# davidmilligan/MLVFS

Hardware: AMD Instinct MI355X
Metric: Mpix/s, 3584x1320 14-bit unpack+badpix+cs5x5+stripes (fused, stream resident in HBM) (higher is better)
Workload: dtype u16/int32

## Files before the change

mlvfs_amd/csrc/k_frame_dev.h:

```cpp
#pragma once
#include "clip.h"
#include <cstdlib>
#include <map>
#include <mutex>
#include <vector>
#include <algorithm>
#include <cstdio>
#include <type_traits>

typedef short mlv_pk16 __attribute__((ext_vector_type(2)));
__device__ __forceinline__ int mlv_min_(int a, int b) { return min(a, b); }
__device__ __forceinline__ int mlv_max_(int a, int b) { return max(a, b); }
__device__ __forceinline__ mlv_pk16 mlv_min_(mlv_pk16 a, mlv_pk16 b) { return __builtin_elementwise_min(a, b); }
__device__ __forceinline__ mlv_pk16 mlv_max_(mlv_pk16 a, mlv_pk16 b) { return __builtin_elementwise_max(a, b); }
#define MLV_NET_FN __device__ __forceinline__
#define mlv_mn(a, b) mlv_min_((a), (b))
#define mlv_mx(a, b) mlv_max_((a), (b))
#include "median_nets.h"


namespace mlv {

constexpr int TCW = FRAME_TCW;
constexpr int TCH = FRAME_TCH;
// ... 770 lines not shown
    for (int c = 0; c < STRIP + 2; c++) {
        const int a = plane[row_top][col_left + c], b = plane[row_top + 1][col_left + c], d = plane[row_top + 2][col_left + c];
        lo[c] = min(min(a, b), d);
        hi[c] = max(max(a, b), d);
        mi[c] = med3i(a, b, d);
    }
#pragma unroll
    for (int c = 0; c < STRIP; c++)
        med[c] = med3i(max(max(lo[c], lo[c + 1]), lo[c + 2]), med3i(mi[c], mi[c + 1], mi[c + 2]),
                       min(min(hi[c], hi[c + 1]), hi[c + 2]));
}

__device__ __forceinline__ void strip_median5(const int (*plane)[PW], int row_top, int col_left, int (&med)[STRIP])
{
#pragma unroll
    for (int c = 0; c < STRIP; c++) {
        const int v[5] = { plane[row_top][col_left + c + 1], plane[row_top + 1][col_left + c],
                           plane[row_top + 1][col_left + c + 1], plane[row_top + 1][col_left + c + 2],
                           plane[row_top + 2][col_left + c + 1] };
        int o[1];
        mlv_median5(v, o);
        med[c] = o[0];
    }
}

template <bool FAST>
__device__ __forceinline__ uint32_t stripe_px(uint32_t p, int coef, int black16, int white16)
{
    if (FAST) {
        const int a = (int)p - black16;
        const int v = (int)p + (__mul24(a, coef - 65536) >> 16);
        return (a > 64) ? (uint32_t)min(v, white16) : p;
    }
    if (coef == 0 || (int)p <= black16 + 64) return p;
    const long long num = (long long)((int)p - black16) * coef + ((long long)black16 << 16);
    if (((long long)white16 << 16) < num) return (uint32_t)white16;
    return (uint32_t)(int)(num / 65536) & 0xFFFFu;
}

template <bool FAST>
__device__ __forceinline__ void stripe_strip(uint32_t (&top)[STRIP], uint32_t (&bot)[STRIP], const int (&coef)[8], int black16, int white16)
{
#pragma unroll
    for (int c = 0; c < STRIP; c++) {
        const int p0 = (2 * c) & 7, p1 = (2 * c + 1) & 7;
        top[c] = stripe_px<FAST>(top[c] & 0xFFFFu, coef[p0], black16, white16) |
                 (stripe_px<FAST>(top[c] >> 16, coef[p1], black16, white16) << 16);
        bot[c] = stripe_px<FAST>(bot[c] & 0xFFFFu, coef[p0], black16, white16) |
                 (stripe_px<FAST>(bot[c] >> 16, coef[p1], black16, white16) << 16);
    }
}

template <bool MASK = true>
__device__ __forceinline__ uint32_t stripe_pair(uint32_t x, int d0, int d1, uint32_t black_pk, uint32_t white_pk)
{
    typedef unsigned short upk16 __attribute__((ext_vector_type(2)));
    const mlv_pk16 a = __builtin_bit_cast(mlv_pk16, x) - __builtin_bit_cast(mlv_pk16, black_pk);
    const mlv_pk16 c64 = { 64, 64 }, s15 = { 15, 15 };
    const int p0 = __mul24((int)a.x, d0), p1 = __mul24((int)a.y, d1);
    const uint32_t delta = __builtin_amdgcn_perm((uint32_t)p1, (uint32_t)p0, 0x07060302u);
    uint32_t dm = delta;
    if (MASK) dm &= __builtin_bit_cast(uint32_t, (c64 - a) >> s15);
    const upk16 v = __builtin_bit_cast(upk16, x) + __builtin_bit_cast(upk16, dm);
    return __builtin_bit_cast(uint32_t, __builtin_elementwise_min(v, __builtin_bit_cast(upk16, white_pk)));
}

template <bool MASK = true>
__device__ __forceinline__ void stripe_strip_pk(uint32_t (&top)[STRIP], uint32_t (&bot)[STRIP], const int (&coef)[8], int black16, int white16)
{
    const uint32_t black_pk = (uint32_t)black16 * 0x10001u, white_pk = (uint32_t)white16 * 0x10001u;
#pragma unroll
    for (int c = 0; c < STRIP; c++) {
        const int d0 = coef[(2 * c) & 7] - 65536, d1 = coef[(2 * c + 1) & 7] - 65536;
        if ((d0 | d1) == 0) {
            typedef unsigned short upk16 __attribute__((ext_vector_type(2)));
            top[c] = __builtin_bit_cast(uint32_t, __builtin_elementwise_min(__builtin_bit_cast(upk16, top[c]), __builtin_bit_cast(upk16, white_pk)));
            bot[c] = __builtin_bit_cast(uint32_t, __builtin_elementwise_min(__builtin_bit_cast(upk16, bot[c]), __builtin_bit_cast(upk16, white_pk)));
            continue;
        }
        top[c] = stripe_pair<MASK>(top[c], d0, d1, black_pk, white_pk);
        bot[c] = stripe_pair<MASK>(bot[c], d0, d1, black_pk, white_pk);
    }
}



typedef const __attribute__((address_space(4))) FrameArgs *KArgs;
__device__ __forceinline__ KArgs cold_args()
{
    KArgs p = (KArgs)__builtin_amdgcn_kernarg_segment_ptr();
    asm volatile("" : "+s"(p));
    return p;
}


template <int BPP>
__device__ __forceinline__ void item_tile_offsets(const ItemLane &L, int l_row, int w, uint32_t &pre_a, uint32_t &pre_b)
{
    constexpr uint32_t GB = (uint32_t)BPP;
    const uint32_t pitch = (uint32_t)(w >> 3) * GB;
    const uint32_t rowoff = __umul24((uint32_t)(2 * l_row), pitch) + 16u;
    pre_a = rowoff + ((uint32_t)((L.xoff_a >> 3) * (int)GB) & L.amask);
    pre_b = rowoff + ((uint32_t)((L.xoff_b >> 3) * (int)GB) & L.amask) + L.boff;
}
template <int BPP, int VEC, class LANE>
__device__ __forceinline__ void issue_tile_rows_pre(uint32_t (&r0)[4], uint32_t (&r1)[4], const uint8_t *frame, unsigned bytes, uint32_t pre_a, uint32_t pre_b,
                                                    LANE lane_of, int w, int h, int tx0, int ty0, int new0)
{
    constexpr uint32_t GB = (uint32_t)BPP;
    const uint32_t pitch = (uint32_t)(w >> 3) * GB;
    const int ybase = ty0 - 2 * HC + 2 * new0;
    uint32_t oa0, ob0, oa1, ob1, S = 0;
    if (VEC != 2 && tx0 >= 8 && tx0 + 2 * TCW + 8 <= w && ybase + 2 * TCH <= h) {
        S = (uint32_t)ybase * pitch + (uint32_t)(tx0 >> 3) * GB - 16u;
        oa0 = pre_a;
        ob0 = pre_b;
        oa1 = oa0 + pitch;
        ob1 = ob0 + pitch;
    } else {
        int l_row;
        const ItemLane L = lane_of(l_row);
        const int y = ybase + 2 * l_row;
        const int gmax = (w >> 3) - 1, g0 = tx0 >> 3;
        const uint32_t ga = __umul24((uint32_t)min(g0 + (L.xoff_a >> 3), gmax), GB);
        const uint32_t gb = __umul24((uint32_t)max(min(g0 + (L.xoff_b >> 3), gmax), 0), GB);
        const uint32_t row0 = __umul24((uint32_t)min(y, h - 1), pitch), row1 = __umul24((uint32_t)min(y + 1, h - 1), pitch);
        oa0 = (row0 + ga) & L.amask; ob0 = ((row0 + gb) & L.amask) + L.boff;
        oa1 = (row1 + ga) & L.amask; ob1 = ((row1 + gb) & L.amask) + L.boff;
        asm volatile("" : "+v"(oa0), "+v"(ob0));
    }
    const mlv_i32x4 rs = frame_rsrc(frame + S, bytes - S);
    const mlv_u32x2 a0 = mlv_rbl_x2(rs, (int)oa0, 0, AUX_DEFAULT), b0 = mlv_rbl_x2(rs, (int)ob0, 0, AUX_DEFAULT);
    const mlv_u32x2 a1 = mlv_rbl_x2(rs, (int)oa1, 0, AUX_DEFAULT), b1 = mlv_rbl_x2(rs, (int)ob1, 0, AUX_DEFAULT);
    r0[0] = a0.x; r0[1] = a0.y; r0[2] = b0.x; r0[3] = b0.y;
    r1[0] = a1.x; r1[1] = a1.y; r1[2] = b1.x; r1[3] = b1.y;
}
template <int BPP, int VEC>
__device__ __forceinline__ void issue_tile_rows(uint32_t (&r0)[4], uint32_t (&r1)[4], const uint8_t *frame, unsigned bytes, const ItemLane &L, int l_row,
                                                int w, int h, int tx0, int ty0, int new0)
{
    uint32_t pre_a, pre_b;
    item_tile_offsets<BPP>(L, l_row, w, pre_a, pre_b);
    issue_tile_rows_pre<BPP, VEC>(r0, r1, frame, bytes, pre_a, pre_b, [&](int &row) { row = l_row; return L; }, w, h, tx0, ty0, new0);
}

struct OutArgs {
    const uint2 *e2d;
    uint8_t *dst;
    size_t dst_stride;
    int stripes, coef_pk, coef_fast, white;
    int co[8];
};
__device__ __forceinline__ OutArgs out_args(KArgs kt)
{
    OutArgs o;
    o.e2d = kt->e2d; o.dst = kt->dst; o.dst_stride = kt->dst_stride;
    o.stripes = kt->stripes; o.coef_pk = kt->coef_pk; o.coef_fast = kt->coef_fast; o.white = kt->white;
#pragma unroll
    for (int i = 0; i < 8; i++) o.co[i] = kt->coef[i];
    return o;
}

__device__ __forceinline__ void put_rb(uint32_t &top, uint32_t &bot, uint32_t ur, uint32_t ub, unsigned long long m)
{
    asm("s_mov_b64 vcc, %4\n\t"
        "v_cndmask_b32_sdwa %0, %0, %2, vcc dst_sel:WORD_0 dst_unused:UNUSED_PRESERVE src0_sel:WORD_0 src1_sel:WORD_0\n\t"
        "v_cndmask_b32_sdwa %1, %1, %3, vcc dst_sel:WORD_1 dst_unused:UNUSED_PRESERVE src0_sel:WORD_1 src1_sel:WORD_0"
        : "+v"(top), "+v"(bot) : "v"(ur), "v"(ub), "s"(m) : "vcc");
}
__device__ __forceinline__ unsigned long long lanes_gt(int a, int b) { return __builtin_amdgcn_sicmp(a, b, 38); }
__device__ __forceinline__ unsigned long long lanes_ge(int a, int b) { return __builtin_amdgcn_sicmp(a, b, 39); }
__device__ __forceinline__ unsigned long long lanes_lt(int a, int b) { return __builtin_amdgcn_sicmp(a, b, 40); }

struct NoSmem {};
__device__ __forceinline__ bool smoothed_low(const int (&er)[STRIP], const int (&eb)[STRIP])
{
    const int lo = min(min(min(min(er[0], er[1]), er[2]), min(er[3], eb[0])), min(min(eb[1], eb[2]), eb[3]));
    return __any(lo < 7 * MLV_EV_RES);
}
template <int METHOD, bool PACKED, bool VECST, bool CLAMP, bool XM, bool ANYSTRIPES, bool BRIGHT, class SM, bool RAWREG = false>
__device__ __forceinline__ void strip_output_t(const SM &sm, const OutArgs &oa, int w, int h, int black, int f, int tx0, int ty0, int jj, int kk,
                                               unsigned long long msmooth, const int (&gev)[STRIP], int gev_off, const int (&er)[STRIP], const int (&eb)[STRIP], bool store,
                                               uint32_t *rtop = nullptr, uint32_t *rbot = nullptr)
{
    const int y = ty0 + 2 * jj, x = tx0 + 2 * STRIP * kk;
    uint32_t top[STRIP], bot[STRIP];
    auto read_raw = [&]() {
        if constexpr (RAWREG) {
#pragma unroll
            for (int c = 0; c < STRIP; c++) { top[c] = rtop[c]; bot[c] = rbot[c]; }
        } else {
            const uint4 v0 = *(const uint4 *)&sm.raw[2 * jj][2 * STRIP * kk];
            const uint4 v1 = *(const uint4 *)&sm.raw[2 * jj + 1][2 * STRIP * kk];
            top[0] = v0.x; top[1] = v0.y; top[2] = v0.z; top[3] = v0.w;
            bot[0] = v1.x; bot[1] = v1.y; bot[2] = v1.z; bot[3] = v1.w;
        }
    };
    if (METHOD == 0) read_raw();
    if (METHOD != 0) {
        const mlv_i32x4 rs_e2d = table_rsrc(oa.e2d, 8, E2D_RECORDS_EXT);
        int ur[STRIP], ub[STRIP], cr[STRIP], cb[STRIP];
        mlv_tab_u32x2 dr2[STRIP], db2[STRIP];
#pragma unroll
        for (int c = 0; c < STRIP; c++) {
            cr[c] = CLAMP ? min(max(er[c], 0), MLV_EV_MAX) : er[c];
            cb[c] = CLAMP ? min(max(eb[c], 0), MLV_EV_MAX) : eb[c];
            dr2[c] = mlv_sbl_x2(rs_e2d, cr[c] >> 5, 0, 0, AUX_DEFAULT);
            db2[c] = mlv_sbl_x2(rs_e2d, cb[c] >> 5, 0, 0, AUX_DEFAULT);
        }
        read_raw();
        asm volatile("" :: "v"(dr2[0]), "v"(dr2[1]), "v"(dr2[2]), "v"(dr2[3]), "v"(db2[0]), "v"(db2[1]), "v"(db2[2]), "v"(db2[3]));
#pragma unroll
        for (int c = 0; c < STRIP; c++) {
            ur[c] = (int)(__builtin_popcount(bfe_low_bits(dr2[c].y, (uint32_t)cr[c])) + dr2[c].x);
            ub[c] = (int)(__builtin_popcount(bfe_low_bits(db2[c].y, (uint32_t)cb[c])) + db2[c].x);
        }
#pragma unroll
        for (int c = 0; c < STRIP; c++) {
            unsigned long long okm = msmooth;
            if (!BRIGHT) okm &= lanes_ge((int)((uint32_t)gev[c] - (uint32_t)gev_off), 2 * MLV_EV_RES) & lanes_gt(er[c], MLV_EV_RES) & lanes_gt(eb[c], MLV_EV_RES);
            if (XM) okm &= lanes_ge(x + 2 * c, 4) & lanes_lt(x + 2 * c, w - 4);
            put_rb(top[c], bot[c], (uint32_t)ur[c], (uint32_t)ub[c], okm);
        }
    }
    if (oa.stripes) {
        const int black16 = (int)(uint16_t)black, white16 = (int)(uint16_t)oa.white;
        if (!ANYSTRIPES) stripe_strip_pk<CLAMP>(top, bot, oa.co, black16, white16);
        else if (PACKED && oa.coef_pk) stripe_strip_pk<true>(top, bot, oa.co, black16, white16);
        else if (oa.coef_fast) stripe_strip<true>(top, bot, oa.co, black16, white16);
        else stripe_strip<false>(top, bot, oa.co, black16, white16);
    }
    if constexpr (RAWREG) {
#pragma unroll
        for (int c = 0; c < STRIP; c++) { rtop[c] = top[c]; rbot[c] = bot[c]; }
    }
    if (store && y < h) {
        if (VECST) {
            if (x < w) {
                const uint32_t T = ((uint32_t)ty0 * (uint32_t)w + (uint32_t)tx0) * 2u;
                const mlv_i32x4 rs_out = frame_rsrc(oa.dst + (size_t)f * oa.dst_stride + T, (uint32_t)w * (uint32_t)h * 2u - T);
                const uint32_t vo = (__umul24((uint32_t)(2 * jj), (uint32_t)w) + 2 * STRIP * (uint32_t)kk) * 2u;
                const mlv_u32x4 vt = { top[0], top[1], top[2], top[3] }, vb = { bot[0], bot[1], bot[2], bot[3] };
                mlv_rbs_x4(vt, rs_out, (int)vo, 0, 2);
                if (y + 1 < h) mlv_rbs_x4(vb, rs_out, (int)vo, w * 2, 2);
            }
        } else {
            uint16_t *out = (uint16_t *)(oa.dst + (size_t)f * oa.dst_stride);
#pragma unroll 1
            for (int c = 0; c < STRIP; c++) {
                const int xc = x + 2 * c;
                if (xc < w) out[(size_t)y * w + xc] = (uint16_t)top[c];
                if (xc + 1 < w) out[(size_t)y * w + xc + 1] = (uint16_t)(top[c] >> 16);
                if (y + 1 < h) {
                    if (xc < w) out[(size_t)(y + 1) * w + xc] = (uint16_t)bot[c];
                    if (xc + 1 < w) out[(size_t)(y + 1) * w + xc + 1] = (uint16_t)(bot[c] >> 16);
                }
            }
        }
    }
}

template <int METHOD, bool PACKED, bool VECST, class SM>
__device__ __forceinline__ void strip_output(const SM &sm, const OutArgs &oa, int w, int h, int black, int f, int tx0, int ty0, int jj, int kk,
                                             unsigned long long msmooth, const int (&gev)[STRIP], int gev_off, const int (&er)[STRIP], const int (&eb)[STRIP], bool low_any, bool bright,
                                             bool store)
{
    const bool xm = tx0 < 4 || tx0 + 2 * TCW > w - 4;
    if (METHOD != 0 && !low_any && oa.stripes && smoothed_low(er, eb)) { low_any = true; bright = false; }
    if (oa.stripes && !(PACKED && oa.coef_pk)) {
        strip_output_t<METHOD, PACKED, VECST, true, true, true, false, SM>(sm, oa, w, h, black, f, tx0, ty0, jj, kk, msmooth, gev, gev_off, er, eb, store);
    } else if (low_any) {
        if (xm) strip_output_t<METHOD, PACKED, VECST, true, true, false, false, SM>(sm, oa, w, h, black, f, tx0, ty0, jj, kk, msmooth, gev, gev_off, er, eb, store);
        else strip_output_t<METHOD, PACKED, VECST, true, false, false, false, SM>(sm, oa, w, h, black, f, tx0, ty0, jj, kk, msmooth, gev, gev_off, er, eb, store);
    } else if (xm) {
        strip_output_t<METHOD, PACKED, VECST, false, true, false, false, SM>(sm, oa, w, h, black, f, tx0, ty0, jj, kk, msmooth, gev, gev_off, er, eb, store);
    } else {
        if (bright) strip_output_t<METHOD, PACKED, VECST, false, false, false, true, SM>(sm, oa, w, h, black, f, tx0, ty0, jj, kk, msmooth, gev, gev_off, er, eb, store);
        else strip_output_t<METHOD, PACKED, VECST, false, false, false, false, SM>(sm, oa, w, h, black, f, tx0, ty0, jj, kk, msmooth, gev, gev_off, er, eb, store);
    }
}

template <int N> using IntC = std::integral_constant<int, N>;
template <class F>
void with_layout(int method, bool packed, int vec, bool spread, F &&f)
{
    auto with_v = [&](auto M, auto P) {
        auto go = [&](auto V) { if (spread && M.value != 0) f(M, P, V, std::true_type{}); else f(M, P, V, std::false_type{}); };
        switch (vec) {
            case 1: return go(IntC<1>{});
            case 2: return go(IntC<2>{});
            case 3: if constexpr (P.value) return go(IntC<3>{}); break;
            case 4: if constexpr (P.value) return go(IntC<4>{}); break;
        }
        go(IntC<0>{});
    };
    auto with_p = [&](auto M) { if (packed) with_v(M, std::true_type{}); else with_v(M, std::false_type{}); };
    switch (method) {
        case 0: return with_p(IntC<0>{});
        case 2: return with_p(IntC<2>{});
        case 3: return with_p(IntC<3>{});
        case 5: return with_p(IntC<5>{});
    }
}

}
```

mlvfs_amd/csrc/k_frame_p.hip:

```cpp
#include "frame_plan.h"
#include "k_stream_dev.h"

namespace mlv {

constexpr int P_WAIT_MIN = 1, P_WAIT_MAX = 15;
template <bool SPREAD_>
struct __align__(16) SmemP {
    static constexpr bool SPREAD = SPREAD_;
    uint16_t raw[2 * RH][2 * TCW];
    uint32_t pk[PH][PW];
    int ge[RH][TCW];
    uint16_t t16[MLV_T16_N + (SPREAD_ ? 64 : 0)];
    uint32_t has_patch[PMAP_WORDS];
    uint32_t xchg[3][XCHG_WORDS];
    int unc[2];
    int low[2];
    int dim[2];
    int next_tile, next_end;
    int walk[5];
    int2 carry_at[256];
    uint4 carry_spare;
};

struct PGroup {
    mlv_pk16 s[4][5];
    mlv_pk16 p0[10], p1[10];
    mlv_pk16 q[6];
};
struct PNext { mlv_pk16 s0[5], s2[5], p0[10], q[6]; };

__device__ __forceinline__ mlv_pk16 as_pk(uint32_t v) { return __builtin_bit_cast(mlv_pk16, v); }
__device__ __forceinline__ uint32_t as_u(mlv_pk16 v) { return __builtin_bit_cast(uint32_t, v); }

__device__ __forceinline__ void pchain_group(const uint32_t (*pk)[PW], int row_top, int col_left, PGroup &g)
{
    mlv_pk16 col[4][5];
#pragma unroll
    for (int r = 0; r < 5; r++) {
        const uint4 v = *(const uint4 *)&pk[row_top + r][col_left];
        col[0][r] = as_pk(v.x); col[1][r] = as_pk(v.y); col[2][r] = as_pk(v.z); col[3][r] = as_pk(v.w);
    }
#pragma unroll
    for (int c = 0; c < 4; c++) mlv_sort5(col[c], g.s[c]);
    mlv_merge55(g.s[0], g.s[1], g.p0);
    mlv_merge55(g.s[2], g.s[3], g.p1);
}
__device__ __forceinline__ void pchain_fetch_lists(const PGroup &g, PNext &n)
{
#pragma unroll
    for (int i = 0; i < 5; i++) { n.s0[i] = dpp_next(g.s[0][i]); n.s2[i] = dpp_next(g.s[2][i]); }
#pragma unroll
    for (int i = 0; i < 10; i++) n.p0[i] = dpp_next(g.p0[i]);
}
__device__ __forceinline__ void pchain_fetch_window(const PGroup &g, PNext &n)
{
#pragma unroll
    for (int i = 0; i < 6; i++) n.q[i] = dpp_next(g.q[i]);
}
__device__ __forceinline__ void pchain_publish(const PGroup &g, uint32_t *x)
{
    uint4 *o = (uint4 *)x;
    o[0] = make_uint4(as_u(g.s[0][0]), as_u(g.s[0][1]), as_u(g.s[0][2]), as_u(g.s[0][3]));
    o[1] = make_uint4(as_u(g.s[0][4]), as_u(g.s[2][0]), as_u(g.s[2][1]), as_u(g.s[2][2]));
    o[2] = make_uint4(as_u(g.s[2][3]), as_u(g.s[2][4]), as_u(g.p0[0]), as_u(g.p0[1]));
    o[3] = make_uint4(as_u(g.p0[2]), as_u(g.p0[3]), as_u(g.p0[4]), as_u(g.p0[5]));
    o[4] = make_uint4(as_u(g.p0[6]), as_u(g.p0[7]), as_u(g.p0[8]), as_u(g.p0[9]));
    o[5] = make_uint4(as_u(g.q[0]), as_u(g.q[1]), as_u(g.q[2]), as_u(g.q[3]));
    *(uint2 *)&o[6] = make_uint2(as_u(g.q[4]), as_u(g.q[5]));
}
__device__ __forceinline__ void pchain_collect_lists(const uint32_t *x, PNext &n)
{
    const uint4 *o = (const uint4 *)x;
    const uint4 a0 = o[0], a1 = o[1], a2 = o[2], a3 = o[3], a4 = o[4];
    n.s0[0] = as_pk(a0.x); n.s0[1] = as_pk(a0.y); n.s0[2] = as_pk(a0.z); n.s0[3] = as_pk(a0.w); n.s0[4] = as_pk(a1.x);
    n.s2[0] = as_pk(a1.y); n.s2[1] = as_pk(a1.z); n.s2[2] = as_pk(a1.w); n.s2[3] = as_pk(a2.x); n.s2[4] = as_pk(a2.y);
    n.p0[0] = as_pk(a2.z); n.p0[1] = as_pk(a2.w); n.p0[2] = as_pk(a3.x); n.p0[3] = as_pk(a3.y); n.p0[4] = as_pk(a3.z);
    n.p0[5] = as_pk(a3.w); n.p0[6] = as_pk(a4.x); n.p0[7] = as_pk(a4.y); n.p0[8] = as_pk(a4.z); n.p0[9] = as_pk(a4.w);
}
__device__ __forceinline__ void pchain_collect_window(const uint32_t *x, PNext &n)
{
    const uint4 a5 = *(const uint4 *)(x + 20);
    const uint2 a6 = *(const uint2 *)(x + 24);
    n.q[0] = as_pk(a5.x); n.q[1] = as_pk(a5.y); n.q[2] = as_pk(a5.z); n.q[3] = as_pk(a5.w); n.q[4] = as_pk(a6.x); n.q[5] = as_pk(a6.y);
}
__device__ __forceinline__ void pchain_finish(const PGroup &g, const PNext &n, mlv_pk16 (&o)[STRIP])
{
    mlv_pk16 q1[6], t[1];
    mlv_quad_mid6(g.p1, n.p0, q1);
    mlv_final6of11(g.q, n.s0, t);  o[0] = t[0];
    mlv_final6of11(q1, g.s[1], t); o[1] = t[0];
    mlv_final6of11(q1, n.s2, t);   o[2] = t[0];
    mlv_final6of11(n.q, g.s[3], t); o[3] = t[0];
}
__device__ __forceinline__ bool pk_uncertain(const mlv_pk16 (&o)[STRIP])
{
    typedef unsigned short upk16 __attribute__((ext_vector_type(2)));
    const upk16 off = { 32769, 32769 }, two = { 2, 2 };
    upk16 m = __builtin_bit_cast(upk16, o[0]) + off;
#pragma unroll
    for (int c = 1; c < STRIP; c++) m = __builtin_elementwise_min(m, (upk16)(__builtin_bit_cast(upk16, o[c]) + off));
    return __builtin_bit_cast(uint32_t, __builtin_elementwise_min(m, two)) != 0x00020002u;
}

__device__ __forceinline__ uint32_t add3_u32(uint32_t a, uint32_t b, uint32_t c)
{
    uint32_t r;
    asm("v_add3_u32 %0, %1, %2, %3" : "=v"(r) : "v"(a), "v"(b), "v"(c));
    return r;
}
template <int NC, bool SPREAD>
__device__ __forceinline__ void cell_multi_pk_fast(const uint32_t *p0, const uint32_t *p1, int black, const uint16_t *t, int ref_r, int ref_b,
                                                   int (&ge)[NC], uint32_t (&pk)[NC])
{
    uint32_t fb[4 * NC], tv[4 * NC];
    const float fmagic = 8388608.0f + (float)black;
#pragma unroll
    for (int c = 0; c < NC; c++) {
        const uint32_t px[4] = { p0[2 * c], p0[2 * c + 1], p1[2 * c], p1[2 * c + 1] };
#pragma unroll
        for (int i = 0; i < 4; i++) fb[4 * c + i] = __float_as_uint(__uint_as_float(px[i] | 0x4B000000u) - fmagic);
    }
#pragma unroll
    for (int i = 0; i < 4 * NC; i++) tv[i] = *(const uint16_t *)((const char *)t + t16_offset<SPREAD>(fb[i]));
    uint32_t exr[NC], exb[NC], exg[NC];
#pragma unroll
    for (int c = 0; c < NC; c++) { exr[c] = fb[4 * c] >> 8; exb[c] = fb[4 * c + 3] >> 8; exg[c] = (fb[4 * c + 1] + fb[4 * c + 2]) >> 8; }
#pragma unroll
    for (int c = 0; c < NC; c += 2) {
        asm volatile("" :: "v"(exr[c]), "v"(exb[c]), "v"(exg[c]), "v"(exr[c + 1]), "v"(exb[c + 1]), "v"(exg[c + 1]));
    }
#pragma unroll
    for (int i = 0; i < 4 * NC; i += 8) {
        asm volatile("" :: "v"(tv[i]), "v"(tv[i + 1]), "v"(tv[i + 2]), "v"(tv[i + 3]), "v"(tv[i + 4]), "v"(tv[i + 5]), "v"(tv[i + 6]), "v"(tv[i + 7]));
    }
    uint32_t nref_r = 0u - (uint32_t)ref_r, nref_b = 0u - (uint32_t)ref_b;
    asm("" : "+v"(nref_r), "+v"(nref_b));
#pragma unroll
    for (int c = 0; c < NC; c++) {
        const uint32_t gb = add3_u32(exg[c], tv[4 * c + 1], tv[4 * c + 2]) >> 1;
        ge[c] = (int)(gb - (127u << 15));
        uint32_t ngr = nref_r - gb, ngb = nref_b - gb;
        pk[c] = as_u(__builtin_amdgcn_cvt_pk_i16((int)add3_u32(exr[c], tv[4 * c + 0], ngr), (int)add3_u32(exb[c], tv[4 * c + 3], ngb)));
    }
}

template <int NC>
__device__ __forceinline__ void cell_multi_pk_tab(const uint32_t *p0, const uint32_t *p1, uint32_t koff, const int *tab, int ref_r, int ref_b,
                                                  int (&ge)[NC], uint32_t (&pk)[NC])
{
    uint32_t ev[4 * NC];
#pragma unroll
    for (int c = 0; c < NC; c++) {
        const uint32_t px[4] = { p0[2 * c], p0[2 * c + 1], p1[2 * c], p1[2 * c + 1] };
#pragma unroll
        for (int i = 0; i < 4; i++) ev[4 * c + i] = *(const uint32_t *)((const char *)tab + ((px[i] << 2) + koff));
    }
#pragma unroll
    for (int i = 0; i < 4 * NC; i += 8) {
        asm volatile("" :: "v"(ev[i]), "v"(ev[i + 1]), "v"(ev[i + 2]), "v"(ev[i + 3]), "v"(ev[i + 4]), "v"(ev[i + 5]), "v"(ev[i + 6]), "v"(ev[i + 7]));
    }
    uint32_t nref_r = 1u - (uint32_t)ref_r, nref_b = 1u - (uint32_t)ref_b;
#pragma unroll
    for (int c = 0; c < NC; c++) {
        const uint32_t gb = (ev[4 * c + 1] + ev[4 * c + 2]) >> 1;
        ge[c] = (int)gb;
        const uint32_t ng = ~gb;
        pk[c] = as_u(__builtin_amdgcn_cvt_pk_i16((int)add3_u32(ev[4 * c + 0], nref_r, ng), (int)add3_u32(ev[4 * c + 3], nref_b, ng)));
    }
}
template <int NC>
__device__ __forceinline__ void cell_multi_pk_tab_dark(const uint32_t *p0, const uint32_t *p1, uint32_t koff, const int *tab, int ref_r, int ref_b,
                                                       int (&ge)[NC], uint32_t (&pk)[NC])
{
    int ev[4 * NC];
#pragma unroll
    for (int c = 0; c < NC; c++) {
        const uint32_t px[4] = { p0[2 * c], p0[2 * c + 1], p1[2 * c], p1[2 * c + 1] };
#pragma unroll
        for (int i = 0; i < 4; i++) ev[4 * c + i] = *(const int *)((const char *)tab + max((int)((px[i] << 2) + koff), 0));
    }
#pragma unroll
    for (int i = 0; i < 4 * NC; i += 8) {
        asm volatile("" :: "v"(ev[i]), "v"(ev[i + 1]), "v"(ev[i + 2]), "v"(ev[i + 3]), "v"(ev[i + 4]), "v"(ev[i + 5]), "v"(ev[i + 6]), "v"(ev[i + 7]));
    }
#pragma unroll
// ... 341 lines not shown
#pragma unroll
            for (int c = 0; c < STRIP; c++) {
                er[c] = wadd(wadd(gev[c], ref_r), (int)o[c].x);
                eb[c] = wadd(wadd(gev[c], ref_b), (int)o[c].y);
            }
            strip_output<METHOD, PACKED, true, Smem>(sm, oa, a.w, a.h, a.black, cur.f, tx0, ty0, j, k, lanes_ge(y, 4) & lanes_lt(y, a.h - 5), gev, 0, er, eb, ((low_cur | low_prev) & 1) != 0, (low_cur | low_prev) == 0, true);
        }
        int4 carry = make_int4(0, 0, 0, 0);
        int2 c_at = make_int2(0, 0);
        if (cont_next) {
            c_at = sm.carry_at[tid];
            carry = *(const int4 *)((const char *)&sm + c_at.x);
        }
        lds_barrier();
        const int unc = __builtin_amdgcn_readfirstlane(sm.unc[par]);
        if (cont_next) *(int4 *)((char *)&sm + c_at.y) = carry;
        have_smp = !cont_next;
        if (unc) {
            if (tid == 0) push(t, 1);
            fb_skip = fb_wait;
            fb_wait = min(2 * fb_wait + 1, P_WAIT_MAX);
            cont = false;
        } else {
            fb_wait = P_WAIT_MIN;
            cont = cont_next;
        }
        low_prev = low_cur;
        t = t_next;
        t_end = t_end_next;
        cur = nxt;
        par ^= 1;
    }
    if (tid == 0) {
        KArgs ka = cold_args();
        const int groups = ka->groups;
        int *tickets = ka->tickets;
        if (atomicAdd(&tickets[2 * groups], 1) == (int)gridDim.x - 1)
            for (int i = 0; i <= 2 * groups; i++) tickets[i] = 0;
    }
}

template <bool SPREAD, int VEC>
__global__ __launch_bounds__(1024, 1) void k_frame_p5(const FrameArgs a, int cols, int segs, int seg_rows, int fold, int S_OUT)
{
    static_assert(!SPREAD, "one table layout");
    asm volatile("" : "+s"(cols));
    constexpr int BPP = 14;
    constexpr int WAVES = 16;
    constexpr int SLOTS = 3;
    constexpr int PARK_LANES = 62;
    struct __align__(16) Smem {
        int ev[MLV_EV32_N];
        uint4 park[WAVES][SLOTS][2][PARK_LANES];
    };
    static_assert(sizeof(Smem) <= 160 * 1024, "the CU's LDS");
    __shared__ Smem sm;
    {
        const uint4 *s4 = (const uint4 *)cold_args()->ev32;
        uint4 *d4 = (uint4 *)sm.ev;
        for (int i = (int)threadIdx.x; i < MLV_EV32_N * 4 / 16; i += 64 * WAVES) d4[i] = s4[i];
    }
    __syncthreads();
    const int lane = (int)threadIdx.x & 63;
    const int w = a.w, h = a.h, black = a.black;
    const uint32_t koff = 4u - 4u * (uint32_t)black;
    const int rows = h >> 1;
    const StreamGrid sg = stream_grid(cols, segs, fold);
    const int ntasks = cold_args()->nframes * sg.per_frame;
    const uint32_t pitch = (uint32_t)(w >> 3) * 14u;
    int *tickets = cold_args()->tickets;
    uint4 (*const mypark)[2][PARK_LANES] = sm.park[threadIdx.x >> 6];
    const int plane = min(max(lane - 1, 0), PARK_LANES - 1);
    const bool parks = lane >= 1 && lane <= PARK_LANES;
    for (;;) {
        const int task = stream_draw(tickets, lane);
        if (task >= ntasks) break;
        const StreamTask t = stream_task<VEC>(task, sg, segs, seg_rows, fold, S_OUT, lane, w, rows);
        const int f = t.f, c = t.c, j0 = t.j0, j1 = t.j1, nparts = t.nparts, P = t.P, roff = t.roff;
        KArgs kt = cold_args();
        const uint8_t *const frame = kt->src + (size_t)f * kt->src_stride;
        const mlv_i32x4 rs_in = frame_rsrc(frame, kt->src_bytes);
        mlv_i32x4 rs_out = { 0, 0, 0, 0 };
        int tx0 = 0;
        bool xm = false;
        uint32_t dA0[4], dA1[4], dB0[4], dB1[4];
        auto issue = [&](int r, uint32_t (&d0)[4], uint32_t (&d1)[4]) { stream_issue(rs_in, r, roff, rows, pitch, t.gbyte, d0, d1); };
        issue(j0 - 2, dA0, dA1);
        issue(j0 - 1, dB0, dB1);
        int ref_r, ref_b;
        {
            const int x0 = min(max(8 * (c * S_OUT + S_OUT / 2), 0), (w - 16) & ~1), y0 = min(j0 + j1, (h - 4) & ~1) & ~1;
            const uint32_t px = fetch_clamped<BPP>(frame, w, h, x0 + (lane & 15), y0 + (lane >> 4));
            const int ev = sm.ev[1 + min(max((int)px - black, 1), 16383)];
            constexpr int CX[5] = { 0, 3, 6, 1, 5 }, CY[5] = { 0, 0, 0, 1, 1 };
            int sdr[5], sdb[5];
#pragma unroll
            for (int k = 0; k < 5; k++) {
                const int l0 = 2 * CX[k] + 32 * CY[k];
                const int rr = __builtin_amdgcn_readlane(ev, l0), g1 = __builtin_amdgcn_readlane(ev, l0 + 1);
                const int g2 = __builtin_amdgcn_readlane(ev, l0 + 16), bb = __builtin_amdgcn_readlane(ev, l0 + 17);
                const int gg = (g1 + g2) >> 1;
                sdr[k] = rr - gg; sdb[k] = bb - gg;
            }
            auto med5 = [](const int (&v)[5]) { return med3i(v[4], max(min(v[0], v[1]), min(v[2], v[3])), min(max(v[0], v[1]), max(v[2], v[3]))); };
            ref_r = med5(sdr);
            ref_b = med5(sdb);
        }
        int n_pm = 0, pm_cell = -1;
        uint32_t pm_top = 0, pm_bot = 0;
        bool list_all = false;
        if (kt->patch) {
            KArgs ka = kt;
            const int4 *cells = ka->cells + (size_t)f * ka->n_rec;
            const int *toff = ka->tile_off;
            const int tx_n = ka->tiles_x, ty_n = ka->tiles_y;
            const int cx_lo = 4 * (c * S_OUT - 1), cx_hi = cx_lo + 4 * P;
            const int tc0 = max(cx_lo - HC, 0) / TCW, tc1 = min((cx_hi - 1 + HC) / TCW, tx_n - 1);
            for (int q = 0; q < nparts; q++) {
                const int j0q = j0 + q * seg_rows, j1q = min(j0q + seg_rows, rows);
                if (j0q >= rows) break;
                const int cy_lo = j0q - 2, cy_hi = j1q + 2;
                const int tr0 = max(cy_lo, 0) / TCH, tr1 = min((cy_hi - 1) / TCH, ty_n - 1), ntr = tr1 - tr0 + 1;
                constexpr int MAXTR = 6;
                int my_lo = 0, my_hi = 0;
                if (lane < ntr && lane < MAXTR) { my_lo = toff[(tr0 + lane) * tx_n + tc0]; my_hi = toff[(tr0 + lane) * tx_n + tc1 + 1]; }
                if (ntr > MAXTR) list_all = true;
                int4 rec[MAXTR];
#pragma unroll
                for (int i = 0; i < MAXTR; i++) {
                    const int rb = __builtin_amdgcn_readlane(my_lo, i), re = __builtin_amdgcn_readlane(my_hi, i);
                    rec[i] = (i < ntr && rb + lane < re) ? cells[rb + lane] : make_int4(-1, 0, 0, 0);
                    if (i < ntr && re - rb > 64) list_all = true;
                }
#pragma unroll
                for (int i = 0; i < MAXTR; i++) {
                    const int rcx = rec[i].x & 0xFFFF, rcy = rec[i].x >> 16;
                    const bool in = rec[i].x >= 0 && rcx >= cx_lo && rcx < cx_hi && rcy >= cy_lo && rcy < cy_hi && rcy / TCH == tr0 + i;
                    unsigned long long m = __ballot(in);
                    while (m) {
                        const int src = __builtin_ctzll(m);
                        m &= m - 1;
                        if (n_pm < 64) {
                            const int vx = __builtin_amdgcn_readlane(rec[i].x, src), vy = __builtin_amdgcn_readlane(rec[i].y, src), vz = __builtin_amdgcn_readlane(rec[i].z, src);
                            const int at = (((vx >> 16) - q * seg_rows) << 16) | (4 * P * q + (vx & 0xFFFF) - cx_lo);
                            if (lane == n_pm) { pm_cell = at; pm_top = (uint32_t)vy; pm_bot = (uint32_t)vz; }
                            n_pm++;
                        } else list_all = true;
                    }
                }
            }
        }
        uint32_t pkr[4][4] = {};
        int geA[4] = { 0, 0, 0, 0 }, geB[4] = { 0, 0, 0, 0 };
        int fl1 = 3, fl2 = 3, fl3 = 3, fl4 = 3;
        unsigned long long unc_lanes = 0;
        int unc_r0 = 1 << 30, unc_r1 = -1;
        auto load_row = [&](int r, const uint32_t (&d0)[4], const uint32_t (&d1)[4], auto after_unpack, int (&ge)[4], uint32_t (&pk)[4]) {
            uint32_t p0[8], p1[8];
            unpack8<BPP>(d0, t.sel, t.sel, t.sel, p0);
            unpack8<BPP>(d1, t.sel1, t.sel1, t.sel1, p1);
            after_unpack();
            if (n_pm) {
                unsigned long long m = __ballot(lane < n_pm && (pm_cell >> 16) == r);
                while (m) {
                    const int src = __builtin_ctzll(m);
                    m &= m - 1;
                    const int cell = __builtin_amdgcn_readlane(pm_cell, src);
                    const uint32_t t_ = (uint32_t)__builtin_amdgcn_readlane((int)pm_top, src), b_ = (uint32_t)__builtin_amdgcn_readlane((int)pm_bot, src);
                    const int cxr = cell & 0xFFFF;
                    const bool mine = (cxr >> 2) == lane;
                    const int cc = cxr & 3;
#pragma unroll
                    for (int k = 0; k < 4; k++)
                        if (mine && cc == k) { p0[2 * k] = t_ & 0xFFFFu; p0[2 * k + 1] = t_ >> 16; p1[2 * k] = b_ & 0xFFFFu; p1[2 * k + 1] = b_ >> 16; }
                }
            }
            bool dark;
            const int fl0 = stream_row_low(p0, p1, black, dark);
            if (!dark) cell_multi_pk_tab<4>(p0, p1, koff, sm.ev, ref_r, ref_b, ge, pk);
            else cell_multi_pk_tab_dark<4>(p0, p1, koff, sm.ev, ref_r, ref_b, ge, pk);
            {
                uint4 (&slot)[2][PARK_LANES] = mypark[(unsigned)(r + 2 * SLOTS) % (unsigned)SLOTS];
                if (parks) {
                    slot[0][plane] = make_uint4(p0[0] | (p0[1] << 16), p0[2] | (p0[3] << 16), p0[4] | (p0[5] << 16), p0[6] | (p0[7] << 16));
                    slot[1][plane] = make_uint4(p1[0] | (p1[1] << 16), p1[2] | (p1[3] << 16), p1[4] | (p1[5] << 16), p1[6] | (p1[7] << 16));
                }
            }
            return fl0;
        };
        auto sort_common = [&](const uint32_t (&ra)[4], const uint32_t (&rb)[4], const uint32_t (&rc)[4], const uint32_t (&rd)[4], mlv_pk16 (&c4)[4][4]) {
#pragma unroll
            for (int cc = 0; cc < 4; cc++) {
                const mlv_pk16 v[4] = { as_pk(ra[cc]), as_pk(rb[cc]), as_pk(rc[cc]), as_pk(rd[cc]) };
                mlv_sort4(v, c4[cc]);
            }
        };
        auto finish_row = [&](int jr, const mlv_pk16 (&c4)[4][4], const uint32_t (&x)[4], int fl, const int (&gej)[4], auto hook) {
            const int y = 2 * jr, yl = y + 2 * roff;
            KArgs ke = cold_args();
            const uint2 *const e2d_early = ke->e2d;
            const int stripes_early = ke->stripes;
            const unsigned long long msmooth = lanes_ge(yl, 4) & lanes_lt(yl, h - 5);
            const bool smooth_row = y + 2 * (nparts - 1) * seg_rows >= 4 && y < h - 5;
            mlv_pk16 o[STRIP] = { { 0, 0 }, { 0, 0 }, { 0, 0 }, { 0, 0 } };
            if (smooth_row) {
                PGroup gq;
#pragma unroll
                for (int cc = 0; cc < 4; cc++) {
                    const mlv_pk16 xv[1] = { as_pk(x[cc]) };
                    mlv_insert4(c4[cc], xv, gq.s[cc]);
                }
                mlv_merge55(gq.s[0], gq.s[1], gq.p0);
                mlv_merge55(gq.s[2], gq.s[3], gq.p1);
                mlv_quad_mid6(gq.p0, gq.p1, gq.q);
                PNext n;
                pchain_fetch_lists(gq, n);
                pchain_fetch_window(gq, n);
                mlv_pk16 oc[STRIP];
                pchain_finish(gq, n, oc);
                o[0] = as_pk((uint32_t)dpp_prev_i((int)as_u(oc[2]))); o[1] = as_pk((uint32_t)dpp_prev_i((int)as_u(oc[3])));
                o[2] = oc[0]; o[3] = oc[1];
                const unsigned long long um = __ballot(t.writes && pk_uncertain(o)) & msmooth;
                if (um) { unc_lanes |= um; unc_r0 = min(unc_r0, jr); unc_r1 = max(unc_r1, jr); }
            }
            int er[STRIP], eb[STRIP];
#pragma unroll
            for (int cc = 0; cc < STRIP; cc++) {
                er[cc] = wadd(wadd(gej[cc], ref_r), (int)o[cc].x);
                eb[cc] = wadd(wadd(gej[cc], ref_b), (int)o[cc].y);
            }
            uint32_t top[STRIP], bot[STRIP];
            {
                const uint4 (&slot)[2][PARK_LANES] = mypark[(unsigned)(jr + 2 * SLOTS) % (unsigned)SLOTS];
                const uint4 t4 = slot[0][plane], b4 = slot[1][plane];
                top[0] = t4.x; top[1] = t4.y; top[2] = t4.z; top[3] = t4.w;
                bot[0] = b4.x; bot[1] = b4.y; bot[2] = b4.z; bot[3] = b4.w;
            }
            OutArgs oa = out_args(cold_args());
            oa.e2d = e2d_early; oa.stripes = stripes_early;
            stream_output<5>(oa, t, tx0, xm, rs_out, w, h, black, jr, yl, msmooth, fl, gej, er, eb, top, bot, hook);
        };
        auto named_as_used = [](const uint32_t (&n0)[4], const uint32_t (&n1)[4]) {
            asm volatile("" :: "v"(n0[0]), "v"(n0[1]), "v"(n0[2]), "v"(n0[3]), "v"(n1[0]), "v"(n1[1]), "v"(n1[2]), "v"(n1[3]));
        };
        auto pair_step = [&](auto OUT, int r) {
            int ge0[4], ge1[4];
            uint32_t pk0[4], pk1[4];
            mlv_pk16 c4[4][4];
            auto early_a = [&] { if constexpr (!OUT.value) issue(r + 2, dA0, dA1); };
            auto early_b = [&] { if constexpr (!OUT.value) issue(r + 3, dB0, dB1); };
            auto late_a = [&] { named_as_used(dB0, dB1); issue(r + 2, dA0, dA1); };
            auto late_b = [&] { named_as_used(dA0, dA1); issue(r + 3, dB0, dB1); };
            const int f0 = load_row(r, dA0, dA1, early_a, ge0, pk0);
            if constexpr (OUT.value) {
                sort_common(pkr[1], pkr[2], pkr[3], pk0, c4);
                finish_row(r - 2, c4, pkr[0], f0 | fl1 | fl2 | fl3 | fl4, geA, late_a);
            }
            const int f1 = load_row(r + 1, dB0, dB1, early_b, ge1, pk1);
            if constexpr (OUT.value) finish_row(r - 1, c4, pk1, f1 | f0 | fl1 | fl2 | fl3, geB, late_b);
#pragma unroll
            for (int i = 0; i < 4; i++) { pkr[0][i] = pkr[2][i]; pkr[1][i] = pkr[3][i]; pkr[2][i] = pk0[i]; pkr[3][i] = pk1[i]; geA[i] = ge0[i]; geB[i] = ge1[i]; }
            fl4 = fl2; fl3 = fl1; fl2 = f0; fl1 = f1;
        };
        auto single_step = [&](int r, const uint32_t (&d0)[4], const uint32_t (&d1)[4]) {
            int ge0[4];
            uint32_t pk0[4];
            mlv_pk16 c4[4][4];
            const int f0 = load_row(r, d0, d1, [] {}, ge0, pk0);
            sort_common(pkr[1], pkr[2], pkr[3], pk0, c4);
            finish_row(r - 2, c4, pkr[0], f0 | fl1 | fl2 | fl3 | fl4, geA, StreamNoHook());
#pragma unroll
            for (int i = 0; i < 4; i++) { pkr[0][i] = pkr[1][i]; pkr[1][i] = pkr[2][i]; pkr[2][i] = pkr[3][i]; pkr[3][i] = pk0[i]; geA[i] = geB[i]; geB[i] = ge0[i]; }
            fl4 = fl3; fl3 = fl2; fl2 = fl1; fl1 = f0;
        };
        constexpr std::true_type Y{};
        constexpr std::false_type N{};
        int r = j0 - 2;
#pragma unroll 1
        for (; r < j0 + 2; r += 2) pair_step(N, r);
        named_as_used(dA0, dA1);
        {
            KArgs ko = cold_args();
            rs_out = frame_rsrc(ko->dst + (size_t)f * ko->dst_stride, (uint32_t)w * (uint32_t)h * 2u);
            tx0 = 8 * (c * S_OUT - 1);
            xm = c == 0 || 8 * (c * S_OUT + S_OUT) > w - 4;
        }
#pragma unroll 1
        for (; r < j1; r += 2) pair_step(Y, r);
#pragma unroll 1
        for (bool second = false; r <= j1 + 1; r++, second = true) {
            uint32_t e0[4], e1[4];
#pragma unroll
            for (int i = 0; i < 4; i++) { e0[i] = second ? dB0[i] : dA0[i]; e1[i] = second ? dB1[i] : dA1[i]; }
            single_step(r, e0, e1);
        }
        if (list_all) { unc_lanes = ~0ull; unc_r0 = j0; unc_r1 = j1 - 1; }
        if (unc_lanes && lane == 0) {
            KArgs kl = cold_args();
            const int tnx = kl->tiles_x, tny = kl->tiles_y;
            int *ctl = kl->wl_ctl;
            for (int q = 0; q < nparts; q++) {
                const unsigned long long mq = P == 64 ? unc_lanes : (unc_lanes >> (q * P)) & ((1ull << P) - 1);
                const int r0 = unc_r0 + q * seg_rows, r1 = min(unc_r1 + q * seg_rows, rows - 1);
                if (!mq || r0 >= rows) continue;
                const int l0 = __builtin_ctzll(mq), l1 = 63 - __builtin_clzll(mq);
                const int cx0 = max(4 * (c * S_OUT + l0 - 1), 0), cx1 = min(4 * (c * S_OUT + l1 - 1) + 3, w / 2 - 1);
                const int tc0 = cx0 / TCW, tc1 = min(cx1 / TCW, tnx - 1), tr0 = r0 / TCH, tr1 = min(r1 / TCH, tny - 1);
                for (int tc = tc0; tc <= tc1; tc++) {
                    const int i = atomicAdd(&ctl[0], 1);
                    kl->wl[i] = make_int2(f * tnx * tny + tc * tny + tr0, tr1 - tr0 + 1);
                    atomicAdd(&ctl[3], tr1 - tr0 + 1);
                }
            }
        }
    }
    stream_last_out(tickets, lane, WAVES, [] {});
}

void launch_frame_p(const FramePlan &pl, int method, bool packed, int vec, bool spread, hipStream_t stream, const FrameArgs &a)
{
#ifdef KFP_ONLY
    hipLaunchKernelGGL((k_frame_p<true, 1, false>), dim3(pl.first_grid), dim3(256), 0, stream, a);
#else
    with_layout(method, packed, vec, spread, [&](auto M, auto P, auto V, auto S) {
        if constexpr (M.value == 5 && P.value && (V.value == 1 || V.value == 2)) {
            if (pl.first == FirstKernel::p5) {
                hipLaunchKernelGGL((k_frame_p5<false, V.value>), dim3((pl.first_grid + 3) / 4), dim3(1024), 0, stream, a, pl.cols, pl.segs, pl.seg_rows,
                                   pl.fold, FRAME_STREAM_COLW);
                return;
            }
        }
        if constexpr (M.value == 5 && V.value != 0)
            hipLaunchKernelGGL((k_frame_p<P.value, V.value, S.value>), dim3(pl.first_grid), dim3(256), 0, stream, a);
    });
#endif
}

void preload_k_frame_p() { hipFuncAttributes fa; (void)hipFuncGetAttributes(&fa, (const void *)k_frame_p<true, 1, false>); (void)hipGetLastError(); }

}
```

mlvfs_amd/csrc/k_stream_dev.h:

```cpp
#pragma once
#include "k_frame_dev.h"

namespace mlv {

struct StreamGrid { int ncols_full, nfolded, per_frame; };
__device__ __forceinline__ StreamGrid stream_grid(int cols, int segs, int fold)
{
    StreamGrid sg;
    sg.ncols_full = fold > 1 ? cols - 1 : cols;
    sg.nfolded = fold > 1 ? (segs + fold - 1) / fold : 0;
    sg.per_frame = sg.ncols_full * segs + sg.nfolded;
    return sg;
}

__device__ __forceinline__ int stream_draw(int *tickets, int lane)
{
    int task = 0;
    if (lane == 0) task = atomicAdd(&tickets[0], 1);
    return __builtin_amdgcn_readfirstlane(task);
}

struct StreamTask {
    int f, c;
    int j0, j1;
    int nparts, P;
    int pl, part, roff;
    int g;
    bool writes;
    uint32_t gbyte;
    uint32_t sel, sel1;
};
template <int VEC>
__device__ __forceinline__ StreamTask stream_task(int task, const StreamGrid &sg, int segs, int seg_rows, int fold, int S_OUT, int lane, int w, int rows)
{
    StreamTask t;
    const int gmax = (w >> 3) - 1;
    t.f = task / sg.per_frame;
    const int rem = task - t.f * sg.per_frame;
    const bool folded = rem >= sg.ncols_full * segs;
    t.c = folded ? sg.ncols_full : rem / segs;
    const int seg = folded ? (rem - sg.ncols_full * segs) * fold : rem - t.c * segs;
    t.j0 = seg * seg_rows; t.j1 = min(t.j0 + seg_rows, rows);
    t.nparts = folded ? fold : 1; t.P = folded ? 64 / fold : 64;
    t.pl = lane & (t.P - 1); t.part = folded ? lane / t.P : 0;
    t.roff = t.part * seg_rows;
    const int g_true = t.c * S_OUT + t.pl - 1;
    t.g = min(max(g_true, 0), gmax);
    t.writes = t.pl >= 1 && t.pl <= min(S_OUT, t.P - 2) && g_true <= gmax && t.j0 + t.roff < rows;
    t.gbyte = (uint32_t)t.g * 14u;
    t.sel = (t.g & 1) ? SEL_MIS : SEL_SWAP;
    t.sel1 = VEC == 2 ? t.sel ^ (SEL_SWAP ^ SEL_MIS) : t.sel;
    return t;
}

__device__ __forceinline__ void stream_issue(mlv_i32x4 rs_in, int r, int roff, int rows, uint32_t pitch, uint32_t gbyte, uint32_t (&d0)[4], uint32_t (&d1)[4])
{
    const int rr = min(max(r + roff, 0), rows - 1);
    const uint32_t o0u = __umul24((uint32_t)(2 * rr), pitch) + gbyte, o0 = o0u & ~3u, o1 = (o0u + pitch) & ~3u;
    const mlv_u32x2 a0 = mlv_rbl_x2(rs_in, (int)o0, 0, AUX_DEFAULT), b0 = mlv_rbl_x2(rs_in, (int)o0 + 8, 0, AUX_DEFAULT);
    const mlv_u32x2 a1 = mlv_rbl_x2(rs_in, (int)o1, 0, AUX_DEFAULT), b1 = mlv_rbl_x2(rs_in, (int)o1 + 8, 0, AUX_DEFAULT);
    d0[0] = a0.x; d0[1] = a0.y; d0[2] = b0.x; d0[3] = b0.y;
    d1[0] = a1.x; d1[1] = a1.y; d1[2] = b1.x; d1[3] = b1.y;
}

__device__ __forceinline__ int stream_row_low(const uint32_t (&p0)[8], const uint32_t (&p1)[8], int black, bool &dark)
{
    uint32_t lo = min(p0[0], p1[0]);
#pragma unroll
    for (int i = 1; i < 8; i++) lo = min(min(lo, p0[i]), p1[i]);
    dark = __any((int)lo <= black);
    int fl = 0;
    if (__any((int)lo <= black + 255)) fl = __any((int)lo <= black + 64) ? 3 : 2;
    return fl;
}

struct StreamNoHook { __device__ __forceinline__ void operator()() const {} };
template <int METHOD, class BEFORE_STORES = StreamNoHook>
__device__ __forceinline__ void stream_output(const OutArgs &oa, const StreamTask &t, int tx0, bool xm, mlv_i32x4 rs_out, int w, int h, int black, int jr, int yl,
                                              unsigned long long msmooth, int fl, const int (&ge)[STRIP], const int (&er)[STRIP], const int (&eb)[STRIP],
                                              uint32_t (&top)[STRIP], uint32_t (&bot)[STRIP], BEFORE_STORES before_stores = BEFORE_STORES())
{
    fl |= oa.stripes && smoothed_low(er, eb) ? 1 : 0;
    auto out = [&](auto CLAMP, auto XM, auto BRIGHT) {
        strip_output_t<METHOD, true, true, CLAMP.value, XM.value, false, BRIGHT.value, NoSmem, true>(NoSmem(), oa, w, h, black, t.f, tx0, 0, jr, t.pl, msmooth,
                                                                                                     ge, 0, er, eb, false, top, bot);
    };
    constexpr std::true_type Y{};
    constexpr std::false_type N{};
    if (fl & 1) { if (xm) out(Y, Y, N); else out(Y, N, N); }
    else if (xm) out(N, Y, N);
    else if (fl == 0) out(N, N, Y);
    else out(N, N, N);
    before_stores();
    if (t.writes) {
        const uint32_t vo = (__umul24((uint32_t)yl, (uint32_t)w) + (uint32_t)(8 * t.g)) * 2u;
        const mlv_u32x4 vt = { top[0], top[1], top[2], top[3] }, vb = { bot[0], bot[1], bot[2], bot[3] };
        mlv_rbs_x4(vt, rs_out, (int)vo, 0, 2);
        mlv_rbs_x4(vb, rs_out, (int)vo, w * 2, 2);
    }
}

template <class AFTER>
__device__ __forceinline__ void stream_last_out(int *tickets, int lane, int waves_per_wg, AFTER after)
{
    if (lane == 0) {
        const int nwaves = (int)gridDim.x * waves_per_wg;
        if (atomicAdd(&tickets[1], 1) == nwaves - 1) {
            tickets[0] = 0; tickets[1] = 0;
            after();
        }
    }
}

}
```

Baseline: 975,800.

## Streamline stream output dispatch with scalar lane masks and an all-replace fast path

```diff
diff --git a/mlvfs_amd/csrc/k_frame_dev.h b/mlvfs_amd/csrc/k_frame_dev.h
--- a/mlvfs_amd/csrc/k_frame_dev.h
+++ b/mlvfs_amd/csrc/k_frame_dev.h
@@ -876,6 +876,27 @@
         bot[c] = stripe_pair<MASK>(bot[c], d0, d1, black_pk, white_pk);
     }
 }
+template <bool MASK = true>
+__device__ __forceinline__ void stripe_strip_pk_steps(uint32_t (&top)[STRIP], uint32_t (&bot)[STRIP], const int (&coef)[8], int black16, int white16)
+{
+    typedef unsigned short upk16 __attribute__((ext_vector_type(2)));
+    const uint32_t black_pk = (uint32_t)black16 * 0x10001u, white_pk = (uint32_t)white16 * 0x10001u;
+    auto corrected = [&](uint32_t x, int d0, int d1) {
+        const mlv_pk16 a = __builtin_bit_cast(mlv_pk16, x) - __builtin_bit_cast(mlv_pk16, black_pk);
+        const mlv_pk16 c64 = { 64, 64 }, s15 = { 15, 15 };
+        const int p0 = __mul24((int)a.x, d0), p1 = __mul24((int)a.y, d1);
+        uint32_t dm = __builtin_amdgcn_perm((uint32_t)p1, (uint32_t)p0, 0x07060302u);
+        if (MASK) dm &= __builtin_bit_cast(uint32_t, (c64 - a) >> s15);
+        return __builtin_bit_cast(uint32_t, (upk16)(__builtin_bit_cast(upk16, x) + __builtin_bit_cast(upk16, dm)));
+    };
+#pragma unroll
+    for (int c = 0; c < STRIP; c++) {
+        const int d0 = coef[(2 * c) & 7] - 65536, d1 = coef[(2 * c + 1) & 7] - 65536;
+        if ((d0 | d1) != 0) { top[c] = corrected(top[c], d0, d1); bot[c] = corrected(bot[c], d0, d1); }
+        top[c] = __builtin_bit_cast(uint32_t, __builtin_elementwise_min(__builtin_bit_cast(upk16, top[c]), __builtin_bit_cast(upk16, white_pk)));
+        bot[c] = __builtin_bit_cast(uint32_t, __builtin_elementwise_min(__builtin_bit_cast(upk16, bot[c]), __builtin_bit_cast(upk16, white_pk)));
+    }
+}
 
 
 
@@ -965,6 +986,20 @@
 __device__ __forceinline__ unsigned long long lanes_gt(int a, int b) { return __builtin_amdgcn_sicmp(a, b, 38); }
 __device__ __forceinline__ unsigned long long lanes_ge(int a, int b) { return __builtin_amdgcn_sicmp(a, b, 39); }
 __device__ __forceinline__ unsigned long long lanes_lt(int a, int b) { return __builtin_amdgcn_sicmp(a, b, 40); }
+__device__ __forceinline__ unsigned long long lanes_eq(int a, int b) { return __builtin_amdgcn_sicmp(a, b, 32); }
+__device__ __forceinline__ unsigned long long lanes_ne(int a, int b) { return __builtin_amdgcn_sicmp(a, b, 33); }
+__device__ __forceinline__ int lanes_any(unsigned long long m)
+{
+    int r;
+    asm("s_cmp_lg_u64 %1, 0\n\ts_cselect_b32 %0, 1, 0" : "=s"(r) : "s"(m) : "scc");
+    return r;
+}
+__device__ __forceinline__ int lanes_all(unsigned long long m)
+{
+    int r;
+    asm("s_cmp_eq_u64 %1, -1\n\ts_cselect_b32 %0, 1, 0" : "=s"(r) : "s"(m) : "scc");
+    return r;
+}
 
 struct NoSmem {};
 __device__ __forceinline__ bool smoothed_low(const int (&er)[STRIP], const int (&eb)[STRIP])
@@ -1009,6 +1044,23 @@
             ur[c] = (int)(__builtin_popcount(bfe_low_bits(dr2[c].y, (uint32_t)cr[c])) + dr2[c].x);
             ub[c] = (int)(__builtin_popcount(bfe_low_bits(db2[c].y, (uint32_t)cb[c])) + db2[c].x);
         }
+        int replace_all = 0;
+        if constexpr (RAWREG && BRIGHT && !XM) {
+            replace_all = lanes_all(msmooth);
+            int ra = replace_all;
+            asm volatile("" : "+s"(ra));
+            if (ra) {
+#pragma unroll
+                for (int c = 0; c < STRIP; c++) {
+                    typedef unsigned short upk16 __attribute__((ext_vector_type(2)));
+                    const upk16 t2 = { (unsigned short)ur[c], (unsigned short)(top[c] >> 16) };
+                    const upk16 b2 = { (unsigned short)bot[c], (unsigned short)ub[c] };
+                    top[c] = __builtin_bit_cast(uint32_t, t2);
+                    bot[c] = __builtin_bit_cast(uint32_t, b2);
+                }
+            }
+        }
+        if (!replace_all)
 #pragma unroll
         for (int c = 0; c < STRIP; c++) {
             unsigned long long okm = msmooth;
@@ -1019,7 +1071,10 @@
     }
     if (oa.stripes) {
         const int black16 = (int)(uint16_t)black, white16 = (int)(uint16_t)oa.white;
-        if (!ANYSTRIPES) stripe_strip_pk<CLAMP>(top, bot, oa.co, black16, white16);
+        if (!ANYSTRIPES) {
+            if constexpr (RAWREG) stripe_strip_pk_steps<CLAMP>(top, bot, oa.co, black16, white16);
+            else stripe_strip_pk<CLAMP>(top, bot, oa.co, black16, white16);
+        }
         else if (PACKED && oa.coef_pk) stripe_strip_pk<true>(top, bot, oa.co, black16, white16);
         else if (oa.coef_fast) stripe_strip<true>(top, bot, oa.co, black16, white16);
         else stripe_strip<false>(top, bot, oa.co, black16, white16);
diff --git a/mlvfs_amd/csrc/k_frame_p.hip b/mlvfs_amd/csrc/k_frame_p.hip
--- a/mlvfs_amd/csrc/k_frame_p.hip
+++ b/mlvfs_amd/csrc/k_frame_p.hip
@@ -92,15 +92,17 @@
     mlv_final6of11(q1, n.s2, t);   o[2] = t[0];
     mlv_final6of11(n.q, g.s[3], t); o[3] = t[0];
 }
-__device__ __forceinline__ bool pk_uncertain(const mlv_pk16 (&o)[STRIP])
+__device__ __forceinline__ uint32_t pk_least2(const mlv_pk16 (&o)[STRIP])
 {
     typedef unsigned short upk16 __attribute__((ext_vector_type(2)));
     const upk16 off = { 32769, 32769 }, two = { 2, 2 };
     upk16 m = __builtin_bit_cast(upk16, o[0]) + off;
 #pragma unroll
     for (int c = 1; c < STRIP; c++) m = __builtin_elementwise_min(m, (upk16)(__builtin_bit_cast(upk16, o[c]) + off));
-    return __builtin_bit_cast(uint32_t, __builtin_elementwise_min(m, two)) != 0x00020002u;
-}
+    return __builtin_bit_cast(uint32_t, __builtin_elementwise_min(m, two));
+}
+__device__ __forceinline__ bool pk_uncertain(const mlv_pk16 (&o)[STRIP]) { return pk_least2(o) != 0x00020002u; }
+__device__ __forceinline__ unsigned long long pk_uncertain_lanes(const mlv_pk16 (&o)[STRIP]) { return lanes_ne((int)pk_least2(o), 0x00020002); }
 
 __device__ __forceinline__ uint32_t add3_u32(uint32_t a, uint32_t b, uint32_t c)
 {
@@ -608,7 +610,7 @@
         const mlv_i32x4 rs_in = frame_rsrc(frame, kt->src_bytes);
         mlv_i32x4 rs_out = { 0, 0, 0, 0 };
         int tx0 = 0;
-        bool xm = false;
+        int xm = 0;
         uint32_t dA0[4], dA1[4], dB0[4], dB1[4];
         auto issue = [&](int r, uint32_t (&d0)[4], uint32_t (&d1)[4]) { stream_issue(rs_in, r, roff, rows, pitch, t.gbyte, d0, d1); };
         issue(j0 - 2, dA0, dA1);
@@ -687,7 +689,7 @@
             unpack8<BPP>(d1, t.sel1, t.sel1, t.sel1, p1);
             after_unpack();
             if (n_pm) {
-                unsigned long long m = __ballot(lane < n_pm && (pm_cell >> 16) == r);
+                unsigned long long m = lanes_lt(lane, n_pm) & lanes_eq(pm_cell >> 16, r);
                 while (m) {
                     const int src = __builtin_ctzll(m);
                     m &= m - 1;
@@ -746,7 +748,8 @@
                 pchain_finish(gq, n, oc);
                 o[0] = as_pk((uint32_t)dpp_prev_i((int)as_u(oc[2]))); o[1] = as_pk((uint32_t)dpp_prev_i((int)as_u(oc[3])));
                 o[2] = oc[0]; o[3] = oc[1];
-                const unsigned long long um = __ballot(t.writes && pk_uncertain(o)) & msmooth;
+                unsigned long long um = pk_uncertain_lanes(o) & msmooth;
+                if (um) um &= __ballot(t.writes);
                 if (um) { unc_lanes |= um; unc_r0 = min(unc_r0, jr); unc_r1 = max(unc_r1, jr); }
             }
             int er[STRIP], eb[STRIP];
@@ -809,7 +812,7 @@
             KArgs ko = cold_args();
             rs_out = frame_rsrc(ko->dst + (size_t)f * ko->dst_stride, (uint32_t)w * (uint32_t)h * 2u);
             tx0 = 8 * (c * S_OUT - 1);
-            xm = c == 0 || 8 * (c * S_OUT + S_OUT) > w - 4;
+            xm = (c == 0 || 8 * (c * S_OUT + S_OUT) > w - 4) ? 1 : 0;
         }
 #pragma unroll 1
         for (; r < j1; r += 2) pair_step(Y, r);
diff --git a/mlvfs_amd/csrc/k_stream_dev.h b/mlvfs_amd/csrc/k_stream_dev.h
--- a/mlvfs_amd/csrc/k_stream_dev.h
+++ b/mlvfs_amd/csrc/k_stream_dev.h
@@ -76,21 +76,29 @@
 
 struct StreamNoHook { __device__ __forceinline__ void operator()() const {} };
 template <int METHOD, class BEFORE_STORES = StreamNoHook>
-__device__ __forceinline__ void stream_output(const OutArgs &oa, const StreamTask &t, int tx0, bool xm, mlv_i32x4 rs_out, int w, int h, int black, int jr, int yl,
+__device__ __forceinline__ void stream_output(const OutArgs &oa, const StreamTask &t, int tx0, int xm, mlv_i32x4 rs_out, int w, int h, int black, int jr, int yl,
                                               unsigned long long msmooth, int fl, const int (&ge)[STRIP], const int (&er)[STRIP], const int (&eb)[STRIP],
                                               uint32_t (&top)[STRIP], uint32_t (&bot)[STRIP], BEFORE_STORES before_stores = BEFORE_STORES())
 {
-    fl |= oa.stripes && smoothed_low(er, eb) ? 1 : 0;
+    if (oa.stripes) {
+        const int lo = min(min(min(min(er[0], er[1]), er[2]), min(er[3], eb[0])), min(min(eb[1], eb[2]), eb[3]));
+        fl |= lanes_any(lanes_lt(lo, 7 * MLV_EV_RES));
+    }
+    OutArgs ob = oa;
+    asm("" : "+s"(ob.stripes));
     auto out = [&](auto CLAMP, auto XM, auto BRIGHT) {
-        strip_output_t<METHOD, true, true, CLAMP.value, XM.value, false, BRIGHT.value, NoSmem, true>(NoSmem(), oa, w, h, black, t.f, tx0, 0, jr, t.pl, msmooth,
+        strip_output_t<METHOD, true, true, CLAMP.value, XM.value, false, BRIGHT.value, NoSmem, true>(NoSmem(), ob, w, h, black, t.f, tx0, 0, jr, t.pl, msmooth,
                                                                                                      ge, 0, er, eb, false, top, bot);
     };
     constexpr std::true_type Y{};
     constexpr std::false_type N{};
-    if (fl & 1) { if (xm) out(Y, Y, N); else out(Y, N, N); }
-    else if (xm) out(N, Y, N);
-    else if (fl == 0) out(N, N, Y);
-    else out(N, N, N);
+    const int variant = __builtin_amdgcn_readfirstlane((fl & 1) ? 1 - xm : xm ? 2 : fl == 0 ? 4 : 3);
+    auto is = [&](int k) { int v = variant; asm volatile("" : "+s"(v)); return v == k; };
+    if (is(0)) out(Y, Y, N);
+    if (is(1)) out(Y, N, N);
+    if (is(2)) out(N, Y, N);
+    if (is(3)) out(N, N, N);
+    if (is(4)) out(N, N, Y);
     before_stores();
     if (t.writes) {
         const uint32_t vo = (__umul24((uint32_t)yl, (uint32_t)w) + (uint32_t)(8 * t.g)) * 2u;
```

Result: no change. 984,900, median of 6 (+0.9%).
